# RaikoPipe/panda-gym

Measured on AMD Instinct MI355X. Metric: aggregate env-steps/s, PandaReach 4096 envs @1 GPU; 1/2/4/8-GPU scaling, higher is better.
Workload: dtype f32; 1 GPU; PandaReach-v3 (ee control, sparse reward), 4096 envs per GPU, the reference's scene: table / plane contacts of the robot (BASELINE configs[1]); envs_per_gpu=4096, global_envs=4096, parallelism=env-sharded x1

## Files before the change

panda-gym_amd/csrc/pgx_kernels.hip:

```cpp
#include <hip/hip_runtime.h>
#include <math.h>
#include <stdint.h>

#include "../../include/pgx.h"
#include "pgx_default_model.h"
#include "pgx_common.h"
#include "pgx_dev.h"
#include "pgx_model_consts.h"
#include "pgx_rows.h"

#ifdef PGX_PROF
#define PGX_PROF_N 24
__device__ unsigned long long pgx_prof_counters[PGX_PROF_N];
#define PGX_PROF_WAVES 16384
__device__ unsigned long long pgx_prof_wave[PGX_PROF_WAVES][10];
extern "C" int pgx_prof_wave_read(unsigned long long* out, int n) {
    return (int)hipMemcpyFromSymbol(out, HIP_SYMBOL(pgx_prof_wave), sizeof(unsigned long long) * 10 * (size_t)n);
}
extern "C" int pgx_prof_read(unsigned long long* out, int clear) {
    hipError_t e = hipMemcpyFromSymbol(out, HIP_SYMBOL(pgx_prof_counters), sizeof(unsigned long long) * PGX_PROF_N);
    if (e == hipSuccess && clear) {
        unsigned long long z[PGX_PROF_N] = {0};
        e = hipMemcpyToSymbol(HIP_SYMBOL(pgx_prof_counters), z, sizeof z);
    }
// ... 59 lines not shown
            printf("PGX_NAN tag %d sub %d block %d lane %d v %g %g %g %g %g %g %g | dt %g kp %g kd %g "     \
                   "maxv %g res %g erp %g fr %g it %d\n",                                                 \
                   (tag), (sub), (int)blockIdx.x, (int)threadIdx.x, (arr)[0], (n) > 1 ? (arr)[1] : 0.0f,   \
                   (n) > 2 ? (arr)[2] : 0.0f, (n) > 3 ? (arr)[3] : 0.0f, (n) > 4 ? (arr)[4] : 0.0f,        \
                   (n) > 5 ? (arr)[5] : 0.0f, (n) > 6 ? (arr)[6] : 0.0f, (mm).dt, (mm).kp, (mm).kd,         \
                   (mm).max_vel, (mm).residual_abs, (mm).contact_erp, (mm).friction, (mm).num_iterations); \
    } while (0)
#else
#define PGX_TRAP(tag, sub, arr, n, mm) ((void)0)
#endif

struct V3 {
    float x, y, z;
};
__device__ __forceinline__ V3 v3(float x, float y, float z) { return V3{x, y, z}; }
__device__ __forceinline__ V3 operator+(V3 a, V3 b) { return v3(a.x + b.x, a.y + b.y, a.z + b.z); }
__device__ __forceinline__ V3 operator-(V3 a, V3 b) { return v3(a.x - b.x, a.y - b.y, a.z - b.z); }
__device__ __forceinline__ V3 operator*(float s, V3 a) { return v3(s * a.x, s * a.y, s * a.z); }
__device__ __forceinline__ float dot(V3 a, V3 b) { return a.x * b.x + a.y * b.y + a.z * b.z; }
__device__ __forceinline__ V3 cross(V3 a, V3 b) {
    return v3(a.y * b.z - a.z * b.y, a.z * b.x - a.x * b.z, a.x * b.y - a.y * b.x);
}
__device__ __forceinline__ float fast_rcp(float x) { return __builtin_amdgcn_rcpf(x); }
__device__ __forceinline__ float fast_sqrt(float x) { return __builtin_amdgcn_sqrtf(x); }
__device__ __forceinline__ float norm(V3 a) { return fast_sqrt(dot(a, a)); }
__device__ __forceinline__ bool finite3(V3 a) {
    return __builtin_isfinite(a.x) && __builtin_isfinite(a.y) && __builtin_isfinite(a.z);
}

__device__ __forceinline__ void joint_sincos(float x, float* s_out, float* c_out) {
    const float k = rintf(x * 0.63661977236758134f);
    float r = fmaf(k, -1.5703125f, x);
    r = fmaf(k, -4.837512969970703125e-4f, r);
    r = fmaf(k, -7.54978995489188216e-8f, r);
    const float z = r * r;
    const float s = fmaf(r * z, fmaf(z, fmaf(z, -1.9515295891e-4f, 8.3321608736e-3f), -1.6666654611e-1f), r);
    const float c = fmaf(z * z, fmaf(z, fmaf(z, 2.443315711809948e-5f, -1.388731625493765e-3f), 4.166664568298827e-2f),
                         fmaf(-0.5f, z, 1.0f));
    const int q = (int)k & 3;
    const float ss = (q & 1) ? c : s, cc = (q & 1) ? s : c;
    *s_out = (q & 2) ? -ss : ss;
    *c_out = ((q + 1) & 2) ? -cc : cc;
}

template <int W>
__device__ __forceinline__ V3 lds3(const float (*a)[W], int ln) { return v3(a[0][ln], a[1][ln], a[2][ln]); }

typedef float f2 __attribute__((ext_vector_type(2)));
#ifndef PGX_PK
#define PGX_PK 4
#endif
#ifndef PGX_PK_AO
#define PGX_PK_AO 2
#endif
__device__ __forceinline__ void pk_fma_acc(float& a, float& b, f2 cab, float s) {
    const f2 r = __builtin_elementwise_fma(cab, (f2){s, s}, (f2){a, b});
    a = r.x;
    b = r.y;
}
constexpr int GW = 16;
constexpr int EPW = 64 / GW;

template <int V>
struct IC {
    static constexpr int value = V;
};
template <int B, int E, class F>
__device__ __forceinline__ void sfor(F&& f) {
    if constexpr (B < E) {
        f(IC<B>{});
        sfor<B + 1, E>(f);
    }
}
template <int CTRL>
__device__ __forceinline__ float dpp(float x) {
    return __builtin_bit_cast(float, __builtin_amdgcn_update_dpp(0, __builtin_bit_cast(int, x), CTRL, 0xF, 0xF, true));
}
template <int SRC>
__device__ __forceinline__ float bcast16(float x) {
    return dpp<0x150 + SRC>(x);
}
__device__ __forceinline__ float sum16(float x) {
    x += dpp<0xB1>(x);
    x += dpp<0x4E>(x);
    x += dpp<0x141>(x);
    x += dpp<0x140>(x);
    return x;
}
template <int K>
__device__ __forceinline__ float lane_sel(float a, float other) {
    constexpr uint64_t mask = 0x0001000100010001ull << K;
    float r;
    asm("v_cndmask_b32 %0, %1, %2, %3" : "=v"(r) : "v"(other), "v"(a), "s"(mask));
    return r;
}
__device__ __forceinline__ float pick_obj(V3 lin, V3 ang) {
    float v = 0.0f;
    v = lane_sel<7>(lin.x, v); v = lane_sel<8>(lin.y, v); v = lane_sel<9>(lin.z, v);
    v = lane_sel<10>(ang.x, v); v = lane_sel<11>(ang.y, v); v = lane_sel<12>(ang.z, v);
    return v;
}
__device__ __forceinline__ float pick_arm(const float* a, float other) {
    float v = other;
    sfor<0, NJ>([&](auto kc) __attribute__((always_inline)) { v = lane_sel<decltype(kc)::value>(a[decltype(kc)::value], v); });
    return v;
}
// ... 491 lines not shown
#ifndef PGX_CGR_OBJ
#define PGX_CGR_OBJ 6
#endif
#ifndef PGX_CGR_ARM
#define PGX_CGR_ARM 4
#endif
static_assert(PGX_CGR_ARM >= 2 && PGX_CGR_OBJ >= 2, "the sweeps' point counts are 0, 2, 4 (<= the register budget)");
template <int W, int OBJ, int FULL>
constexpr int robot_regs() {
    return (W != 64 && FULL) ? (OBJ ? PGX_CGR_OBJ : PGX_CGR_ARM) : CG;
}

constexpr int CACHE_N = 2 * PGX_CONTACT_SLOTS;
constexpr int CACHE1 = 2 * CG;
constexpr float kTableIdLimit = 32.0f;
static_assert(PGX_NCAP <= 16, "PgxDevModel.cap_mu holds 16 capsules");

template <int AO, int FULL = 0>
__device__ __forceinline__ float point_mu(MRef m, float id) {
    const float cf = id < kTableIdLimit ? id * 0.5f
                   : (id - kTableIdLimit) * (AO ? ((FULL && AO_PERS) ? (1.0f / 24.0f) : (1.0f / 6.0f)) : 0.0625f);
    const int cap = (int)(cf + 1e-3f);
    float mu = m.friction;
    sfor<0, PGX_NCAP>([&](auto kc) __attribute__((always_inline)) {
        constexpr int K = decltype(kc)::value;
        mu = cap == K ? m.cap_mu[K] : mu;
    });
    return mu;
}

template <int W, int OBJ = 1, int FULL = 0>
struct ContactLdsT {
    static constexpr int RB = robot_budget<W, OBJ, FULL>();
    static constexpr int P0 = OBJ ? CG : 0;
    static constexpr int CGR = robot_regs<W, OBJ, FULL>();
    static constexpr int NQR = 3 * (P0 + CGR), NQX = 3 * (P0 + RB);
    static constexpr int XR = (W == 64 || RB <= CGR) ? 1 : NQX - NQR;
    static constexpr int MP = (W == 64 || !FULL) ? 1 : (OBJ ? PGX_MANIFOLD_POOL : PGX_MANIFOLD_POOL_AO);
    static constexpr int G0 = (W == 64 || OBJ) ? CG : 1;
    float4 g0q[G0][4][W];
    float g0d[G0][W], g0id[G0][W];
    float g0n[G0][3][W];
    float g1p[RB][3][W];
    float g1n[RB][3][W];
    float g1rb[RB][3][W];
    float g1d[RB][W], g1id[RB][W];
    int g1j[RB][W];
    int g1w[RB][W];
    int mcnt[W];
    float mkid[MP][W], mla[MP][3][W], mlb[MP][3][W], mn[MP][3][W], md[MP][W], mimp[MP][W];
    float4 g1q[W == 64 ? CG : 1][3][6][W == 64 ? W : 1];
    int cnt[2][W];
    float cache[CACHE_N][W];
    float capA[PGX_NCAP][3][W], capB[PGX_NCAP][3][W];
    float aoC[PGX_AO_OBSTACLES][3][W];
    float aoD[PGX_AO_LINKS][W], aoU[PGX_AO_LINKS][3][W];
    float4 wJ[W == 64 ? 1 : W][W == 64 ? 1 : NQR][4], wR[W == 64 ? 1 : W][W == 64 ? 1 : NQR][2];
    float2 xd[(W == 64 || XR == 1) ? 1 : W][XR][16];
    float xrhs[XR][W], xlam[XR][W], xlam0[XR][W], xfk[XR][W], xjinv[XR][W];
    float pjn[W == 64 ? 1 : P0 + CGR][W], pl0[W == 64 ? 1 : P0 + CGR][W];
    float lrhs[(W == 64 || !OBJ) ? 1 : PGX_N_ROWS - PGX_NJ][W], llam[(W == 64 || !OBJ) ? 1 : PGX_N_ROWS - PGX_NJ][W];
    float ltq[W == 64 ? 1 : PGX_NJ][W], lqs[W == 64 ? 1 : 2][W == 64 ? 1 : PGX_NJ][W];
    float lkc[W == 64 ? 1 : 16][W == 64 ? 1 : 16];
    float psv[W == 64 ? 1 : 27][W == 64 ? 1 : W];
    float spec0[W == 64 ? NJ + 6 : 1][W == 64 ? W : 1];
};
using ContactLds = ContactLdsT<64>;
template <int OBJ, int FULL>
using ContactLdsGT = ContactLdsT<EPW, OBJ, FULL>;

template <int N, class LT>
__device__ __forceinline__ float warm_lookup(const LT& L, int ln, int first, float id, float factor) {
    float warm = 0.0f;
#pragma unroll
    for (int s = 0; s < N; s++) {
        const float sid = L.cache[first + 2 * s][ln], imp = L.cache[first + 2 * s + 1][ln];
        warm = sid == id ? factor * imp : warm;
    }
    return warm;
}

struct ObjState {
    V3 p, v, w;
    float qx, qy, qz, qw;
};

__device__ __forceinline__ void plane_space(V3 n, V3& p, V3& q) {
    if (fabsf(n.z) > 0.70710678f) {
        float a = n.y * n.y + n.z * n.z, k = __builtin_amdgcn_rsqf(a);
        p = v3(0.0f, -n.z * k, n.y * k);
        q = v3(a * k, -n.x * p.z, n.x * p.y);
    } else {
        float a = n.x * n.x + n.y * n.y, k = __builtin_amdgcn_rsqf(a);
        p = v3(-n.y * k, n.x * k, 0.0f);
        q = v3(-n.z * p.y, n.z * p.x, a * k);
    }
}

__device__ __forceinline__ bool on_table(const PgxDevEnv& e, float x, float y) {
    return fabsf(x - e.table_cx) <= e.table_hx && fabsf(y - e.table_cy) <= e.table_hy;
}
__device__ __forceinline__ float ground_z(const PgxDevEnv& e, float x, float y) {
    return on_table(e, x, y) ? e.table_top : e.plane_z;
}
__device__ __forceinline__ float vertex_vs_table(const PgxDevEnv& e, V3 P, V3& n) {
    const float bot = e.table_top - 2.0f * e.table_hz;
    const float qx = P.x - e.table_cx, qy = P.y - e.table_cy;
// ... 537 lines not shown
        const V3 A = v3(L.capA[c][0][ln], L.capA[c][1][ln], L.capA[c][2][ln]);
        const V3 B = v3(L.capB[c][0][ln], L.capB[c][1][ln], L.capB[c][2][ln]);
        const float r = kCapR[c];
        const int flags = kCapFlags[c], jc = kCapJ[c], ns = kCapNs[c];
        if (flags & PGX_CAP_VS_TABLE) {
            for (int end = 0; end < (ns == 1 ? 1 : 2); end++) {
                const V3 P = end ? B : A;
                const bool ont = on_table(e, P.x, P.y);
                const float zt = ont ? e.table_top : e.plane_z;
                const float d = P.z - r - zt;
                if (d < (ont ? cap_tau<TAU_TABLE>(m, c) : cap_tau<TAU_PLANE>(m, c)))
                    g1_insert(L, ln, d, (float)(2 * c + end), jc, v3(P.x, P.y, P.z - r), v3(0.0f, 0.0f, 1.0f),
                              v3(0.0f, 0.0f, 0.0f));
            }
        }
        if (OBJ && (flags & PGX_CAP_VS_OBJECT)) object_candidates(e, cap_tau<TAU_OBJ>(m, c), L, ln, ob, Rc, c, true);
        if (AO && flags != 0) {
            const float tau = cap_tau<TAU_OBST>(m, c);
            if (ao_capsule_near(L, ln, c, tau)) ao_obstacle_candidates(L, ln, c, tau);
        }
    }
}

template <int C = 0, class LT>
__device__ __forceinline__ void link_capsules(int j, LT& L, int ln, const M3& R, V3 oj) {
    if constexpr (C < PGX_NCAP) {
        if (kCapJ[C] == j) {
            const V3 A = oj + mulc(R, kCapA[C]), B = oj + mulc(R, kCapB[C]);
            L.capA[C][0][ln] = A.x; L.capA[C][1][ln] = A.y; L.capA[C][2][ln] = A.z;
            L.capB[C][0][ln] = B.x; L.capB[C][1][ln] = B.y; L.capB[C][2][ln] = B.z;
        }
        link_capsules<C + 1, LT>(j, L, ln, R, oj);
    }
}

struct CapLane {
    float r;
    int flags, ns, j, slot;
};
__device__ __forceinline__ CapLane cap_lane() {
    float r = kCapR[0], fl = (float)kCapFlags[0], ns = (float)kCapNs[0], j = (float)kCapJ[0];
    float sl = (float)ao_slot(0);
    sfor<1, PGX_NCAP>([&](auto kc) __attribute__((always_inline)) {
        constexpr int K = decltype(kc)::value;
        r = lane_sel<K>(kCapR[K], r);
        fl = lane_sel<K>((float)kCapFlags[K], fl);
        ns = lane_sel<K>((float)kCapNs[K], ns);
        j = lane_sel<K>((float)kCapJ[K], j);
        sl = lane_sel<K>((float)ao_slot(K), sl);
    });
    return CapLane{r, (int)fl, (int)ns, (int)j, (int)sl};
}

template <class LT>
__device__ __forceinline__ void robot_table_contacts_g(MRef m, const PgxDevEnv& e, LT& L, int es, int c) {
    const int cc = c < PGX_NCAP ? c : 0;
    const CapLane cl = cap_lane();
    const bool on = c < PGX_NCAP && (cl.flags & PGX_CAP_VS_TABLE);
    const V3 A = lds3(L.capA[cc], es), B = lds3(L.capB[cc], es);
    const float r = cl.r;
    const bool two = cl.ns != 1;
    const float tt = cap_tau<TAU_TABLE>(m, cc), tp = cap_tau<TAU_PLANE>(m, cc);
    const bool t0 = on_table(e, A.x, A.y), t1 = on_table(e, B.x, B.y);
    const float d0 = A.z - r - (t0 ? e.table_top : e.plane_z);
    const float d1 = B.z - r - (t1 ? e.table_top : e.plane_z);
    const bool c0 = on && d0 < (t0 ? tt : tp), c1 = on && two && d1 < (t1 ? tt : tp);
    unsigned m0 = row_ballot(c0), m1 = row_ballot(c1);
    const int total = __builtin_popcount(m0) + __builtin_popcount(m1);
    bool k0 = c0, k1 = c1;
    if (__any(total > LT::RB)) {
        const float e0 = c0 ? d0 : 3.0e38f, e1 = c1 ? d1 : 3.0e38f;
        int r0 = 0, r1 = 0;
        sfor<0, PGX_NCAP>([&](auto kc) __attribute__((always_inline)) {
            constexpr int K = decltype(kc)::value;
            const float y0 = bcast16<K>(e0), y1 = bcast16<K>(e1);
            r0 += (y0 < e0 || (y0 == e0 && K < c)) + (y1 < e0 || (y1 == e0 && K < c));
            r1 += (y0 < e1 || (y0 == e1 && K <= c)) + (y1 < e1 || (y1 == e1 && K < c));
        });
        k0 = c0 && r0 < LT::RB;
        k1 = c1 && r1 < LT::RB;
        m0 = row_ballot(k0);
        m1 = row_ballot(k1);
    }
    const unsigned below = (1u << (c & 15)) - 1u;
    const int base = __builtin_popcount(m0 & below) + __builtin_popcount(m1 & below);
    const int jc = cl.j;
    if (k0) {
        const int sl = base;
        L.g1d[sl][es] = d0; L.g1id[sl][es] = (float)(2 * c); L.g1j[sl][es] = jc; L.g1w[sl][es] = -1;
        L.g1p[sl][0][es] = A.x; L.g1p[sl][1][es] = A.y; L.g1p[sl][2][es] = A.z - r;
        L.g1n[sl][0][es] = 0.0f; L.g1n[sl][1][es] = 0.0f; L.g1n[sl][2][es] = 1.0f;
        L.g1rb[sl][0][es] = 0.0f; L.g1rb[sl][1][es] = 0.0f; L.g1rb[sl][2][es] = 0.0f;
    }
    if (k1) {
        const int sl = base + (k0 ? 1 : 0);
        L.g1d[sl][es] = d1; L.g1id[sl][es] = (float)(2 * c + 1); L.g1j[sl][es] = jc; L.g1w[sl][es] = -1;
        L.g1p[sl][0][es] = B.x; L.g1p[sl][1][es] = B.y; L.g1p[sl][2][es] = B.z - r;
        L.g1n[sl][0][es] = 0.0f; L.g1n[sl][1][es] = 0.0f; L.g1n[sl][2][es] = 1.0f;
        L.g1rb[sl][0][es] = 0.0f; L.g1rb[sl][1][es] = 0.0f; L.g1rb[sl][2][es] = 0.0f;
    }
    L.cnt[1][es] = __builtin_popcount(m0) + __builtin_popcount(m1);
}

struct Dyn {
    V3 z[NJ], o[NJ];
    float Mi[NJ][NJ];
    float mcol[NJ];
    float mdiag[NJ];
    float vu[NJ];
    V3 vcu, wcu;
    bool coll;
};

template <int OBJ, int CONT, class LT, bool PAR = false, int AO = 0>
__device__ __forceinline__ void substep_dyn(MRef m, const PgxDevEnv& e, const float* q, const float* qd,
                                            const ObjState& ob, LT* Lp, int ln, Dyn& D, int lane = 0) {
    M3 Rc;
    if (OBJ) Rc = quat_mat(ob);
    if (CONT) { Lp->cnt[0][ln] = 0; Lp->cnt[1][ln] = 0; }
    if (OBJ) {
        const float h = e.obj_half;
#pragma unroll
        for (int k = 0; k < 16; k++) {
            const int vtx = k & 7;
            const V3 r = mul(Rc, v3((vtx & 1) ? h : -h, (vtx & 2) ? h : -h, (vtx & 4) ? h : -h));
            const V3 P = ob.p + r;
            V3 n = v3(0.0f, 0.0f, 1.0f);
            const float d = k < 8 ? vertex_vs_table(e, P, n) : P.z - e.plane_z;
            if (d < (k < 8 ? m.tau_obj_table : m.tau_obj_plane)) g0_insert(*Lp, ln, d, (float)k, r, n);
        }
    }
    V3 (&z)[NJ] = D.z;
    V3 (&o)[NJ] = D.o;
    V3 c[NJ];
    S3 Iw[NJ];
    M3 R6;
    {
        M3 PR = {{1, 0, 0, 0, 1, 0, 0, 0, 1}};
        V3 PO = v3(m.base[0], m.base[1], m.base[2]);
        float sjs[NJ], cjs[NJ];
        joint_sincos_all<PAR>(q, sjs, cjs);
#pragma unroll
        for (int j = 0; j < NJ; j++) {
            M3 R = mulm(PR, kJr[j]);
            V3 oj = PO + mulc(PR, kJp[j]);
            const float s = sjs[j], cs = cjs[j];
#pragma unroll
            for (int r = 0; r < 3; r++) {
                float a = R.m[r * 3], b = R.m[r * 3 + 1];
                R.m[r * 3] = cs * a + s * b;
                R.m[r * 3 + 1] = -s * a + cs * b;
            }
            z[j] = col(R, 2);
            o[j] = oj;
// ... 93 lines not shown
            for (int i = 0; i < j; i++) Mt[j][i] = dot(z[i], n0 + cross(o[j] - o[i], f));
        }
    }
    chol7(Mt);
    float (&vu)[NJ] = D.vu;
    {
        float qdd[NJ];
        chol7_solve(Mt, nb, qdd);
#pragma unroll
        for (int j = 0; j < NJ; j++) vu[j] = fminf(fmaxf(qd[j] + m.dt * qdd[j], -m.max_vel), m.max_vel);
    }

    PGX_PROF_MARK(15);
    float (&Mi)[NJ][NJ] = D.Mi;
    {
        float X[NJ][NJ];
#pragma unroll
        for (int i = 0; i < NJ; i++) {
            float inv = Mt[i][i];
#pragma unroll
            for (int jj = 0; jj <= i; jj++) {
                float s = (jj == i) ? 1.0f : 0.0f;
#pragma unroll
                for (int kk = jj; kk < i; kk++) s -= Mt[i][kk] * X[kk][jj];
                X[i][jj] = s * inv;
            }
        }
#pragma unroll
        for (int i = 0; i < NJ; i++)
#pragma unroll
            for (int jj = 0; jj <= i; jj++) {
                float s = 0.0f;
#pragma unroll
                for (int l = i; l < NJ; l++) s += X[l][i] * X[l][jj];
                Mi[i][jj] = s;
            }
    }

    V3& vcu = D.vcu;
    V3& wcu = D.wcu;
    vcu = v3(0, 0, 0);
    wcu = v3(0, 0, 0);
    if (OBJ) {
        const float vn = norm(ob.v), wn = norm(ob.w);
        vcu = ob.v + m.dt * (g - (m.lin_damp + m.lin_damp * vn) * ob.v - cross(ob.w, ob.v));
        wcu = ob.w - (m.dt * (m.ang_damp + m.ang_damp * wn)) * ob.w;
    }
}

struct LaneK {
    float mass, com[3];
    float I[6], Iown[6];
};
__device__ __forceinline__ void lane_consts(LaneK& k) {
    k.mass = 0.0f;
#pragma unroll
    for (int t = 0; t < 3; t++) k.com[t] = 0.0f;
#pragma unroll
    for (int t = 0; t < 6; t++) { k.I[t] = 0.0f; k.Iown[t] = 0.0f; }
    sfor<0, NJ>([&](auto jc) __attribute__((always_inline)) {
        constexpr int j = decltype(jc)::value;
        k.mass = lane_sel<j>(kMass[j], k.mass);
#pragma unroll
        for (int t = 0; t < 3; t++) k.com[t] = lane_sel<j>(kCom[j][t], k.com[t]);
#pragma unroll
        for (int t = 0; t < 6; t++) {
            const float a = j < NJ - 1 ? (t < 3 ? kInertia[j < NJ - 1 ? j : 0][t < 3 ? t : 0] : 0.0f) : kI6c[t];
            const float b = j < NJ - 1 ? a : kI6own[t];
            if (a != 0.0f) k.I[t] = lane_sel<j>(a, k.I[t]);
            if (b != 0.0f) k.Iown[t] = lane_sel<j>(b, k.Iown[t]);
        }
    });
}
__device__ __forceinline__ float row_pre(float x) {
    x += dpp<0x111>(x);
    x += dpp<0x112>(x);
    x += dpp<0x114>(x);
    return x;
}
__device__ __forceinline__ float row_suf(float x) {
    x += dpp<0x101>(x);
    x += dpp<0x102>(x);
    x += dpp<0x104>(x);
    return x;
}
__device__ __forceinline__ V3 row_pre(V3 a) { return v3(row_pre(a.x), row_pre(a.y), row_pre(a.z)); }
__device__ __forceinline__ V3 row_suf(V3 a) { return v3(row_suf(a.x), row_suf(a.y), row_suf(a.z)); }
__device__ __forceinline__ float link_only(float x) {
    float r;
    asm("v_cndmask_b32 %0, 0, %1, %2" : "=v"(r) : "v"(x), "s"(0x007F007F007F007Full));
    return r;
}
__device__ __forceinline__ V3 link_only(V3 a) { return v3(link_only(a.x), link_only(a.y), link_only(a.z)); }
__device__ __forceinline__ S3 rot_sym_r(const M3& R, const float* s) {
    const float Sm[9] = {s[0], s[3], s[4], s[3], s[1], s[5], s[4], s[5], s[2]};
    float T[9];
#pragma unroll
    for (int i = 0; i < 3; i++)
#pragma unroll
        for (int j = 0; j < 3; j++)
            T[i * 3 + j] = R.m[i * 3] * Sm[j] + R.m[i * 3 + 1] * Sm[3 + j] + R.m[i * 3 + 2] * Sm[6 + j];
    auto e = [&](int i, int j) { return T[i * 3] * R.m[j * 3] + T[i * 3 + 1] * R.m[j * 3 + 1] + T[i * 3 + 2] * R.m[j * 3 + 2]; };
    S3 o;
    o.xx = e(0, 0); o.yy = e(1, 1); o.zz = e(2, 2); o.xy = e(0, 1); o.xz = e(0, 2); o.yz = e(1, 2);
    return o;
}
__device__ __forceinline__ V3 mul_sym(const float* s, V3 v) {
    return v3(s[0] * v.x + s[3] * v.y + s[4] * v.z, s[3] * v.x + s[1] * v.y + s[5] * v.z,
              s[4] * v.x + s[5] * v.y + s[2] * v.z);
}

template <int OBJ, int CONT, int AO = 0, int FULL = 0>
__device__ __forceinline__ void substep_dyn_g(MRef m, const PgxDevEnv& e, const float* q, const float* qd,
                                              const ObjState& ob, ContactLdsGT<OBJ, FULL>* Lp, int es, Dyn& D, int c,
                                              const LaneK& K, bool check = false) {
    M3 Rc;
    D.coll = false;
    if (OBJ) Rc = quat_mat(ob);
    if (CONT) { Lp->cnt[0][es] = 0; Lp->cnt[1][es] = 0; }
    if (OBJ) {
        const float h = e.obj_half;
        const int vtx = c & 7;
        const V3 r = mul(Rc, v3((vtx & 1) ? h : -h, (vtx & 2) ? h : -h, (vtx & 4) ? h : -h));
        const V3 P = ob.p + r;
        V3 nrm = v3(0.0f, 0.0f, 1.0f);
        const float d = c < 8 ? vertex_vs_table(e, P, nrm) : P.z - e.plane_z;
        const bool cand = d < (c < 8 ? m.tau_obj_table : m.tau_obj_plane);
        const float dd = cand ? d : 3.0e38f;
        int rank = 0;
        sfor<0, 16>([&](auto uc) __attribute__((always_inline)) {
            constexpr int U = decltype(uc)::value;
            const float du = bcast16<U>(dd);
            rank += (du < dd || (du == dd && U < c)) ? 1 : 0;
        });
        const bool keep = cand && rank < CG;
        const unsigned mk = row_ballot(keep);
        const int sl = __builtin_popcount(mk & ((1u << (c & 15)) - 1u));
        if (keep) {
            Lp->g0d[sl][es] = d;
            Lp->g0id[sl][es] = (float)c;
            Lp->g0q[sl][0][es] = make_float4(r.x, r.y, r.z, 0.0f);
            Lp->g0n[sl][0][es] = nrm.x; Lp->g0n[sl][1][es] = nrm.y; Lp->g0n[sl][2][es] = nrm.z;
        }
        Lp->cnt[0][es] = __builtin_popcount(mk);
        PGX_PROF_MARK(19);
    }
    V3 (&z)[NJ] = D.z;
    V3 (&o)[NJ] = D.o;
    M3 Rl = {{0, 0, 0, 0, 0, 0, 0, 0, 0}};
    V3 ol = v3(0, 0, 0);
    {
        M3 PR = {{1, 0, 0, 0, 1, 0, 0, 0, 1}};
        V3 PO = v3(m.base[0], m.base[1], m.base[2]);
        float sjs[NJ], cjs[NJ];
        joint_sincos_all<true>(q, sjs, cjs);
        sfor<0, NJ>([&](auto jc) __attribute__((always_inline)) {
            constexpr int j = decltype(jc)::value;
            M3 R = mulm(PR, kJr[j]);
            V3 oj = PO + mulc(PR, kJp[j]);
            const float sn = sjs[j], cs = cjs[j];
#pragma unroll
            for (int r = 0; r < 3; r++) {
                float a = R.m[r * 3], b = R.m[r * 3 + 1];
                R.m[r * 3] = cs * a + sn * b;
                R.m[r * 3 + 1] = -sn * a + cs * b;
            }
            z[j] = col(R, 2);
            o[j] = oj;
            if constexpr (CONT) link_capsules(j, *Lp, es, R, oj);
#pragma unroll
            for (int t = 0; t < 9; t++) Rl.m[t] = lane_sel<j>(R.m[t], Rl.m[t]);
            ol = v3(lane_sel<j>(oj.x, ol.x), lane_sel<j>(oj.y, ol.y), lane_sel<j>(oj.z, ol.z));
            PR = R;
            PO = oj;
        });
    }
    if (CONT) {
        if constexpr (!OBJ) {
            robot_table_contacts_g(m, e, *Lp, es, c);
            if constexpr (AO) {
                const int cc = c < PGX_NCAP ? c : 0;
                const float tau = cap_tau<TAU_OBST>(m, cc);
                const CapLane cl = cap_lane();
                const bool cap_on = c < PGX_NCAP && cl.flags != 0;
                const int slot = c < PGX_NCAP ? cl.slot : -1;
                const bool chk = check && slot >= 0;
                const V3 A = lds3(Lp->capA[cc], es), B = lds3(Lp->capB[cc], es);
                const float r = cl.r;
                const V3 hcube = v3(kAoSize, kAoSize, kAoSize);
                const int row0 = (int)(threadIdx.x & ~(unsigned)(GW - 1));
                bool sorted = false, hit = false;
                if (chk && slot >= 1) {
                    V3 tc = ao_table_c(e), th = ao_table_h(e);
                    asm volatile("" : "+v"(tc.x), "+v"(tc.y), "+v"(tc.z), "+v"(th.x), "+v"(th.y), "+v"(th.z));
                    const V3 thi = v3(th.x - kAoMargin, th.y - kAoMargin, th.z - kAoMargin);
                    const float lb = fminf(box_sd(A, tc, thi), box_sd(B, tc, thi)) - 0.5f * norm(B - A) - kAoMargin - r;
                    if (lb <= 0.0f) hit = capsule_box_hit(A, B, r, tc, th);
                }
                unsigned cmask = 0;
                int o1 = -1;
                V3 pa1 = v3(0.0f, 0.0f, 0.0f), pb1 = pa1, n1v = pa1;
                float d1 = 0.0f;
                V3 Cs[AO_N];
#pragma unroll
                for (int o = 0; o < AO_N; o++) Cs[o] = lds3(Lp->aoC[o], es);
#ifdef PGX_AB_NO_OBST
                if (true) {} else
#endif
#pragma unroll
                for (int o = 0; o < AO_N; o++) {
                    const V3 C = Cs[o];
                    V3 P = seg_closest(A, B, C);
                    const V3 v = C - P;
                    const float len = norm(v);
                    float d = 3.0e38f;
                    V3 n = len > 0.0f ? fast_rcp(len) * v : v3(0.0f, 0.0f, 1.0f);
                    if (cap_on || chk) {
                        if (o < 3) d = len - r - kAoSize;
                        else if (len - r - kAoCubeBound < (cap_on ? tau : 0.0f))
#ifdef PGX_AB_NO_BOXPAIR
                            d = len - r - kAoCubeBound;
#else
                            d = capsule_box_pair<true>(A, B, r, C, hcube, &P, &n);
#endif
                    }
                    hit = hit || (chk && d <= 0.0f);
                    const bool cand = cap_on && d < tau;
                    if constexpr (FULL && AO_PERS) {
                        cmask |= cand ? (1u << o) : 0u;
                        if (cand && o1 < 0) {
                            o1 = o;
                            pa1 = P + r * n;
// ... 86 lines not shown
            const uint64_t bn = __ballot(near);
            unsigned wm = (unsigned)((bn | (bn >> 16) | (bn >> 32) | (bn >> 48)) & 0xFFFFu);
            if constexpr (FULL) {
                const unsigned rm = row_ballot(near);
                wm = __builtin_amdgcn_readfirstlane(wm);
                while (wm) {
                    const int cn = __builtin_ctz(wm);
                    wm &= wm - 1u;
                    object_new_point_g(e, cap_tau<TAU_OBJ>(m, cn), *Lp, es, ob, Rc, cn, c, ((rm >> cn) & 1u) != 0, Rl, ol);
                }
                if (__any(Lp->mcnt[es] > 0)) man_refresh_insert_g<1, 0>(m, *Lp, es, c, Rl, ol, Rc, ob.p);
                PGX_PROF_MARK(21);
            } else if (wm) {
                const unsigned rm = row_ballot(near);
                sort_g1_by_depth(*Lp, es);
                wm = __builtin_amdgcn_readfirstlane(wm);
                while (wm) {
                    const int cn = __builtin_ctz(wm);
                    wm &= wm - 1u;
                    object_candidates_g(e, cap_tau<TAU_OBJ>(m, cn), *Lp, es, ob, Rc, cn, c, ((rm >> cn) & 1u) != 0);
                }
                PGX_PROF_MARK(21);
                sort_groups(*Lp, es);
            }
        }
    }
    PGX_PROF_MARK(1);
    const V3 g = v3(m.gravity[0], m.gravity[1], m.gravity[2]);
    const V3 base = v3(m.base[0], m.base[1], m.base[2]);
    const V3 zl = col(Rl, 2);
    const V3 ob_l = ol - base;
    const V3 cw = ol + mul(Rl, v3(K.com[0], K.com[1], K.com[2]));
    const V3 cb = cw - base;

    const float qdl = pick_arm(qd, 0.0f);
    const V3 t1 = qdl * zl;
    const V3 w = row_pre(t1);
    const V3 alt = cross(w - t1, t1);
    const V3 al = row_pre(alt);
    const V3 S = row_pre(cross(t1, ob_l));
    const V3 u = cross(w, ob_l) - S;
    const V3 dS = row_pre(cross(alt, ob_l) + cross(t1, u));
    const V3 v = cross(w, cb) - S;
    const V3 a = cross(al, cb) + cross(w, v) - dS;
    const S3 Iw = rot_sym_r(Rl, K.I);
    const V3 Iww = mul(Iw, w);
    const float wn = norm(w);
    const V3 Iow = mul(Rl, mul_sym(K.Iown, mul_t(Rl, w)));
    V3 F = K.mass * (a - g);
    V3 T = mul(Iw, al) + cross(w, Iww) + (m.ang_damp + m.ang_damp * wn) * Iow;
    {
        const V3 Fd = (K.mass * (m.lin_damp + m.lin_damp * norm(v))) * v;
        V3 Fg = v3(0, 0, 0), Tg = v3(0, 0, 0);
#pragma unroll
        for (int b = 0; b < PGX_NDAMP; b++) {
            const V3 rb = mulc(Rl, kDpos[b]);
            const V3 vb = u + cross(w, rb);
            const V3 fd = (kDmass[b] * (m.lin_damp + m.lin_damp * norm(vb))) * vb;
            Fg = Fg + fd;
            Tg = Tg + cross(ol + rb - cw, fd);
        }
        F = F + v3(lane_sel<NJ - 1>(Fg.x, Fd.x), lane_sel<NJ - 1>(Fg.y, Fd.y), lane_sel<NJ - 1>(Fg.z, Fd.z));
        T = T + v3(lane_sel<NJ - 1>(Tg.x, 0.0f), lane_sel<NJ - 1>(Tg.y, 0.0f), lane_sel<NJ - 1>(Tg.z, 0.0f));
    }
    const V3 Fs = row_suf(link_only(F));
    const V3 Ms = row_suf(link_only(T + cross(cb, F)));
    const float nbl = -dot(zl, Ms - cross(ob_l, Fs));
    PGX_PROF_MARK(14);

    float Mt[NJ][NJ], yb[NJ];
    {
        const float ml = link_only(K.mass);
        const S3 st = steiner(ml, cb);
        const float Mc = row_suf(ml);
        const V3 H = row_suf(ml * cb);
        const float Ixx = row_suf(link_only(Iw.xx + st.xx)), Iyy = row_suf(link_only(Iw.yy + st.yy));
        const float Izz = row_suf(link_only(Iw.zz + st.zz)), Ixy = row_suf(link_only(Iw.xy + st.xy));
        const float Ixz = row_suf(link_only(Iw.xz + st.xz)), Iyz = row_suf(link_only(Iw.yz + st.yz));
        const S3 Is = {Ixx, Iyy, Izz, Ixy, Ixz, Iyz};
        const V3 f = cross(zl, H - Mc * ob_l);
        const float Ho = dot(H, ob_l), oz = dot(ob_l, zl), Hz = dot(H, zl), oo = dot(ob_l, ob_l);
        const V3 n = mul(Is, zl) + (Mc * oo - 2.0f * Ho) * zl + oz * H + Hz * ob_l - (Mc * oz) * ob_l;
        float colv[NJ];
#pragma unroll
        for (int i = 0; i < NJ; i++) colv[i] = dot(z[i], n + cross(ol - o[i], f));
        chol7_rows(colv, nbl, Mt, yb);
    }
    float (&vu)[NJ] = D.vu;
    {
        float qdd[NJ];
        chol7_back(Mt, yb, qdd);
#pragma unroll
        for (int j = 0; j < NJ; j++) vu[j] = fminf(fmaxf(qd[j] + m.dt * qdd[j], -m.max_vel), m.max_vel);
    }

    PGX_PROF_MARK(15);
    {
        float y[NJ], x[NJ];
        sfor<0, NJ>([&](auto ic) __attribute__((always_inline)) {
            constexpr int i = decltype(ic)::value;
            float sacc = lane_sel<i>(1.0f, 0.0f);
#pragma unroll
            for (int k = 0; k < i; k++) sacc -= Mt[i][k] * y[k];
            y[i] = sacc * Mt[i][i];
        });
#pragma unroll
        for (int i = NJ - 1; i >= 0; i--) {
            float sacc = y[i];
#pragma unroll
            for (int k = i + 1; k < NJ; k++) sacc -= Mt[k][i] * x[k];
            x[i] = sacc * Mt[i][i];
        }
#pragma unroll
// ... 2185 lines not shown
        L->mcnt[ln] = mc;
        if (c < mc) {
            const float* b = s.man + (size_t)(1 + PGX_MANIFOLD_POINT * c) * N + ii;
            L->mkid[c][ln] = b[0];
#pragma unroll
            for (int t = 0; t < 3; t++) {
                L->mla[c][t][ln] = b[(size_t)(1 + t) * N];
                L->mlb[c][t][ln] = b[(size_t)(4 + t) * N];
                L->mn[c][t][ln] = b[(size_t)(7 + t) * N];
            }
            L->md[c][ln] = b[(size_t)10 * N];
            L->mimp[c][ln] = b[(size_t)11 * N];
        }
    }
    if constexpr (AO) ao_load(s, N, ii, *L, ln);

    const int A = e.action_dim;
    if (CONTROL == 0) {
        float a[3];
#pragma unroll
        for (int c = 0; c < 3; c++) a[c] = fminf(fmaxf(action[(size_t)ii * A + c], -1.0f), 1.0f);
        float qcl[NJ];
#pragma unroll
        for (int j = 0; j < NJ; j++) qcl[j] = s.qc[j * N + ii];
        Chain k;
        fk_chain<WIDE != 0>(m, qcl, k);
        V3 pos = k.o[NJ - 1] + mulc(k.R[NJ - 1], kEeCom);
        V3 tgt = pos + v3(a[0] * m.ee_step, a[1] * m.ee_step, a[2] * m.ee_step);
        tgt.z = fmaxf(0.0f, tgt.z);
        const float torn[4] = {1.0f, 0.0f, 0.0f, 0.0f};
        ik<WIDE != 0>(mp, q, tgt, torn, tq);
        if constexpr (!WIDE) PGX_TRAP(0, 0, tq, NJ, m);
    } else {
#pragma unroll
        for (int j = 0; j < NJ; j++) {
            float a = fminf(fmaxf(action[(size_t)ii * A + j], -1.0f), 1.0f);
            tq[j] = q[j] + a * m.joint_step;
        }
    }

    bool bad_in = false;
    if constexpr (GUARD) {
        bool fin = true;
#pragma unroll
        for (int j = 0; j < NJ; j++)
            fin = fin && __builtin_isfinite(q[j]) && __builtin_isfinite(qd[j]) && __builtin_isfinite(tq[j]);
        if constexpr (OBJ)
            fin = fin && finite3(ob.p) && finite3(ob.v) && finite3(ob.w) && __builtin_isfinite(ob.qx) &&
                  __builtin_isfinite(ob.qy) && __builtin_isfinite(ob.qz) && __builtin_isfinite(ob.qw);
        bad_in = !fin;
    }
    PGX_PROF_MARK(0);
    LaneK lk;
    if constexpr (WIDE) lane_consts(lk);
    const int n_substeps = e.n_substeps;
    bool collided = false;
    float qprev[NJ];
#pragma unroll
    for (int j = 0; j < NJ; j++) qprev[j] = q[j];
    constexpr bool PARK = WIDE && CONT && (OBJ || AO || PART == 2);
    auto lds_st = [&](float* a, float v) __attribute__((always_inline)) { __hip_atomic_store(a, v, __ATOMIC_RELAXED, __HIP_MEMORY_SCOPE_WAVEFRONT); };
    auto lds_ld = [&](float* a) __attribute__((always_inline)) { return __hip_atomic_load(a, __ATOMIC_RELAXED, __HIP_MEMORY_SCOPE_WAVEFRONT); };
    float* lkf = &lk.mass;
    static_assert(sizeof(LaneK) == 16 * sizeof(float), "LaneK layout");
    if constexpr (PARK) {
#pragma unroll
        for (int j = 0; j < NJ; j++) lds_st(&L->ltq[j][ln], tq[j]);
#pragma unroll
        for (int f = 0; f < 16; f++) lds_st(&L->lkc[f][c], lkf[f]);
    }
    int qslot = 0;
    for (int st = 0; st < n_substeps; st++) {
        float qstart[NJ];
        if constexpr (PARK) {
#pragma unroll
            for (int j = 0; j < NJ; j++) {
                lds_st(&L->lqs[st & 1][j][ln], q[j]);
                tq[j] = lds_ld(&L->ltq[j][ln]);
            }
#pragma unroll
            for (int f = 0; f < 16; f++) lkf[f] = lds_ld(&L->lkc[f][c]);
        } else {
#pragma unroll
            for (int j = 0; j < NJ; j++) qstart[j] = q[j];
        }
        if constexpr (WIDE) {
            int cl = c, esl = ln;
            if constexpr (AO) asm volatile("" : "+v"(cl), "+v"(esl));
            if (substep_g<OBJ, CONT, PART, AO, FULL>(mp, e, q, qd, tq, ob, L, esl, cl, lk, AO && st > 0)) {
                collided = true;
                break;
            }
        } else {
            substep<OBJ, CONT, AO>(mp, e, q, qd, tq, ob, L, ln);
        }
        if constexpr (PARK) qslot = st & 1;
        else {
#pragma unroll
            for (int j = 0; j < NJ; j++) qprev[j] = qstart[j];
        }
        if constexpr (AO && !WIDE) {
            ao_caps(*fresh(mp), q, *L, ln);
            if (ao_collided(e, *L, ln)) { collided = true; break; }
        }
    }
    if constexpr (AO && WIDE) {
        if (!collided) {
// ... 653 lines not shown
```

Before: 12.24 million env-steps/s.

## Compute capsule endpoints and damping bodies on idle row lanes via permutes

```diff
diff --git a/panda-gym_amd/csrc/pgx_kernels.hip b/panda-gym_amd/csrc/pgx_kernels.hip
--- a/panda-gym_amd/csrc/pgx_kernels.hip
+++ b/panda-gym_amd/csrc/pgx_kernels.hip
@@ -135,6 +135,12 @@
 #endif
 #ifndef PGX_PK_AO
 #define PGX_PK_AO 2
+#endif
+#ifndef PGX_OWN_CAPS
+#define PGX_OWN_CAPS 1
+#endif
+#ifndef PGX_OWN_DAMP
+#define PGX_OWN_DAMP 1
 #endif
 __device__ __forceinline__ void pk_fma_acc(float& a, float& b, f2 cab, float s) {
     const f2 r = __builtin_elementwise_fma(cab, (f2){s, s}, (f2){a, b});
@@ -732,7 +738,12 @@
     float4 g1q[W == 64 ? CG : 1][3][6][W == 64 ? W : 1];
     int cnt[2][W];
     float cache[CACHE_N][W];
-    float capA[PGX_NCAP][3][W], capB[PGX_NCAP][3][W];
+    union alignas(16) {
+        struct {
+            float capA[PGX_NCAP][3][W], capB[PGX_NCAP][3][W];
+        };
+        float capk[W == 64 ? 1 : GW][12];
+    };
     float aoC[PGX_AO_OBSTACLES][3][W];
     float aoD[PGX_AO_LINKS][W], aoU[PGX_AO_LINKS][3][W];
     float4 wJ[W == 64 ? 1 : W][W == 64 ? 1 : NQR][4], wR[W == 64 ? 1 : W][W == 64 ? 1 : NQR][2];
@@ -1376,15 +1387,100 @@
     return CapLane{r, (int)fl, (int)ns, (int)j, (int)sl};
 }
 
+__device__ __forceinline__ float pmul(float x, float k) { return x * k; }
+__device__ __forceinline__ V3 mull(const M3& A, const float* v) {
+    return v3(pmul(A.m[0], v[0]) + pmul(A.m[1], v[1]) + pmul(A.m[2], v[2]),
+              pmul(A.m[3], v[0]) + pmul(A.m[4], v[1]) + pmul(A.m[5], v[2]),
+              pmul(A.m[6], v[0]) + pmul(A.m[7], v[1]) + pmul(A.m[8], v[2]));
+}
+template <uint64_t MASK>
+__device__ __forceinline__ float mask_sel(float a, float other) {
+    float r;
+    asm("v_cndmask_b32 %0, %1, %2, %3" : "=v"(r) : "v"(other), "v"(a), "s"(MASK));
+    return r;
+}
+template <int N>
+constexpr uint64_t zero_lanes(const float (&T)[N][3], int t, int L0, int K0 = 0) {
+    uint64_t mk = 0;
+    for (int k = K0; k < N; k++)
+        if (T[k][t] == 0.0f) mk |= 0x0001000100010001ull << (L0 + k);
+    return mk;
+}
+template <uint64_t Z0, uint64_t Z1, uint64_t Z2>
+__device__ __forceinline__ void own_cols(M3& R) {
+#pragma unroll
+    for (int r = 0; r < 3; r++) {
+        if constexpr (Z0 != 0) R.m[3 * r] = mask_sel<Z0>(-1.0f, R.m[3 * r]);
+        if constexpr (Z1 != 0) R.m[3 * r + 1] = mask_sel<Z1>(-1.0f, R.m[3 * r + 1]);
+        if constexpr (Z2 != 0) R.m[3 * r + 2] = mask_sel<Z2>(-1.0f, R.m[3 * r + 2]);
+    }
+}
+struct CapEnds {
+    float a[3], b[3];
+};
+__device__ __forceinline__ CapEnds cap_ends_lane() {
+    CapEnds k = {{0.0f, 0.0f, 0.0f}, {0.0f, 0.0f, 0.0f}};
+    sfor<1, PGX_NCAP>([&](auto kc) __attribute__((always_inline)) {
+        constexpr int K = decltype(kc)::value;
+        static_assert(kCapJ[K] >= 0 && kCapJ[K] < NJ, "lane kCapJ[c] of the row holds capsule c's frame");
+#pragma unroll
+        for (int t = 0; t < 3; t++) {
+            if (kCapA[K][t] != 0.0f) k.a[t] = lane_sel<K>(kCapA[K][t], k.a[t]);
+            if (kCapB[K][t] != 0.0f) k.b[t] = lane_sel<K>(kCapB[K][t], k.b[t]);
+        }
+    });
+    return k;
+}
+struct CapRow {
+    CapEnds k;
+    CapLane cl;
+    float tt, tp;
+    int src4;
+};
+typedef float f4 __attribute__((ext_vector_type(4)));
 template <class LT>
-__device__ __forceinline__ void robot_table_contacts_g(MRef m, const PgxDevEnv& e, LT& L, int es, int c) {
+__device__ __forceinline__ void cap_row_fill(MRef m, LT& L, int c) {
+    static_assert(sizeof(L.capk) <= sizeof(L.capA) + sizeof(L.capB), "the rows fit where the end points were");
     const int cc = c < PGX_NCAP ? c : 0;
     const CapLane cl = cap_lane();
+    const CapEnds k = cap_ends_lane();
+    f4* row = reinterpret_cast<f4*>(L.capk[c]);
+    row[0] = (f4){k.a[0], k.a[1], k.a[2], cl.r};
+    row[1] = (f4){k.b[0], k.b[1], k.b[2], __int_as_float(cl.flags | (cl.ns << 8) | ((cl.j + 1) << 16))};
+    row[2] = (f4){cap_tau<TAU_TABLE>(m, cc), cap_tau<TAU_PLANE>(m, cc), __int_as_float((cl.j > 0 ? cl.j : 0) << 2), 0.0f};
+}
+template <class LT>
+__device__ __forceinline__ CapRow cap_row_load(LT& L, int c) {
+    const auto* row = (const volatile __attribute__((address_space(3))) f4*)(L.capk[c]);
+    const f4 a = row[0], b = row[1], t = row[2];
+    const int fl = __float_as_int(b.w);
+    return CapRow{{{a.x, a.y, a.z}, {b.x, b.y, b.z}}, CapLane{a.w, fl & 255, (fl >> 8) & 255, (fl >> 16) - 1, 0},
+                  t.x, t.y, __float_as_int(t.z)};
+}
+__device__ __forceinline__ void cap_ends_own(const M3& Rl, V3 ol, const CapRow& cr, V3& A, V3& B) {
+    static_assert(PGX_NCAP <= GW, "one capsule per lane of the row");
+    constexpr uint64_t ZA0 = zero_lanes(kCapA, 0, 0, 1), ZA1 = zero_lanes(kCapA, 1, 0, 1), ZA2 = zero_lanes(kCapA, 2, 0, 1);
+    static_assert(ZA0 == zero_lanes(kCapB, 0, 0, 1) && ZA1 == zero_lanes(kCapB, 1, 0, 1) && ZA2 == zero_lanes(kCapB, 2, 0, 1),
+                  "both ends of a capsule have the same zero components");
+    const int src = (int)((threadIdx.x & 63u & ~(unsigned)(GW - 1)) << 2) + cr.src4;
+    auto from = [&](float x) __attribute__((always_inline)) {
+        return __builtin_bit_cast(float, __builtin_amdgcn_ds_bpermute(src, __builtin_bit_cast(int, x)));
+    };
+    M3 R;
+#pragma unroll
+    for (int t = 0; t < 9; t++) R.m[t] = from(Rl.m[t]);
+    const V3 o = v3(from(ol.x), from(ol.y), from(ol.z));
+    own_cols<ZA0, ZA1, ZA2>(R);
+    A = o + mull(R, cr.k.a);
+    B = o + mull(R, cr.k.b);
+}
+
+template <class LT>
+__device__ __forceinline__ void robot_table_contacts_g(const PgxDevEnv& e, LT& L, int es, int c, V3 A, V3 B,
+                                                       const CapLane& cl, float tt, float tp) {
     const bool on = c < PGX_NCAP && (cl.flags & PGX_CAP_VS_TABLE);
-    const V3 A = lds3(L.capA[cc], es), B = lds3(L.capB[cc], es);
     const float r = cl.r;
     const bool two = cl.ns != 1;
-    const float tt = cap_tau<TAU_TABLE>(m, cc), tp = cap_tau<TAU_PLANE>(m, cc);
     const bool t0 = on_table(e, A.x, A.y), t1 = on_table(e, B.x, B.y);
     const float d0 = A.z - r - (t0 ? e.table_top : e.plane_z);
     const float d1 = B.z - r - (t1 ? e.table_top : e.plane_z);
@@ -1424,6 +1520,12 @@
         L.g1rb[sl][0][es] = 0.0f; L.g1rb[sl][1][es] = 0.0f; L.g1rb[sl][2][es] = 0.0f;
     }
     L.cnt[1][es] = __builtin_popcount(m0) + __builtin_popcount(m1);
+}
+template <class LT>
+__device__ __forceinline__ void robot_table_contacts_g(MRef m, const PgxDevEnv& e, LT& L, int es, int c) {
+    const int cc = c < PGX_NCAP ? c : 0;
+    robot_table_contacts_g(e, L, es, c, lds3(L.capA[cc], es), lds3(L.capB[cc], es), cap_lane(), cap_tau<TAU_TABLE>(m, cc),
+                           cap_tau<TAU_PLANE>(m, cc));
 }
 
 struct Dyn {
@@ -1623,6 +1725,7 @@
     float mass, com[3];
     float I[6], Iown[6];
 };
+template <bool DAMP = false>
 __device__ __forceinline__ void lane_consts(LaneK& k) {
     k.mass = 0.0f;
 #pragma unroll
@@ -1642,6 +1745,16 @@
             if (b != 0.0f) k.Iown[t] = lane_sel<j>(b, k.Iown[t]);
         }
     });
+    if constexpr (DAMP) {
+        static_assert(PGX_NDAMP <= GW - NJ, "one damping body per idle lane of the row");
+        sfor<0, PGX_NDAMP>([&](auto bc) __attribute__((always_inline)) {
+            constexpr int b = decltype(bc)::value;
+            k.mass = lane_sel<NJ + b>(kDmass[b], k.mass);
+#pragma unroll
+            for (int t = 0; t < 3; t++)
+                if (kDpos[b][t] != 0.0f) k.com[t] = lane_sel<NJ + b>(kDpos[b][t], k.com[t]);
+        });
+    }
 }
 __device__ __forceinline__ float row_pre(float x) {
     x += dpp<0x111>(x);
@@ -1685,6 +1798,7 @@
 __device__ __forceinline__ void substep_dyn_g(MRef m, const PgxDevEnv& e, const float* q, const float* qd,
                                               const ObjState& ob, ContactLdsGT<OBJ, FULL>* Lp, int es, Dyn& D, int c,
                                               const LaneK& K, bool check = false) {
+    constexpr bool OWN_CAPS = PGX_OWN_CAPS && CONT && !OBJ && !AO, OWN_DAMP = PGX_OWN_DAMP && !OBJ && !AO;
     M3 Rc;
     D.coll = false;
     if (OBJ) Rc = quat_mat(ob);
@@ -1738,7 +1852,7 @@
             }
             z[j] = col(R, 2);
             o[j] = oj;
-            if constexpr (CONT) link_capsules(j, *Lp, es, R, oj);
+            if constexpr (CONT && !OWN_CAPS) link_capsules(j, *Lp, es, R, oj);
 #pragma unroll
             for (int t = 0; t < 9; t++) Rl.m[t] = lane_sel<j>(R.m[t], Rl.m[t]);
             ol = v3(lane_sel<j>(oj.x, ol.x), lane_sel<j>(oj.y, ol.y), lane_sel<j>(oj.z, ol.z));
@@ -1748,7 +1862,14 @@
     }
     if (CONT) {
         if constexpr (!OBJ) {
-            robot_table_contacts_g(m, e, *Lp, es, c);
+            if constexpr (OWN_CAPS) {
+                const CapRow cr = cap_row_load(*Lp, c);
+                V3 A, B;
+                cap_ends_own(Rl, ol, cr, A, B);
+                robot_table_contacts_g(e, *Lp, es, c, A, B, cr.cl, cr.tt, cr.tp);
+            } else {
+                robot_table_contacts_g(m, e, *Lp, es, c);
+            }
             if constexpr (AO) {
                 const int cc = c < PGX_NCAP ? c : 0;
                 const float tau = cap_tau<TAU_OBST>(m, cc);
@@ -1941,13 +2062,38 @@
     {
         const V3 Fd = (K.mass * (m.lin_damp + m.lin_damp * norm(v))) * v;
         V3 Fg = v3(0, 0, 0), Tg = v3(0, 0, 0);
-#pragma unroll
-        for (int b = 0; b < PGX_NDAMP; b++) {
-            const V3 rb = mulc(Rl, kDpos[b]);
-            const V3 vb = u + cross(w, rb);
-            const V3 fd = (kDmass[b] * (m.lin_damp + m.lin_damp * norm(vb))) * vb;
-            Fg = Fg + fd;
-            Tg = Tg + cross(ol + rb - cw, fd);
+        if constexpr (OWN_DAMP) {
+            constexpr int S = NJ - 1;
+            constexpr uint64_t Z0 = zero_lanes(kDpos, 0, NJ), Z1 = zero_lanes(kDpos, 1, NJ);
+            static_assert(Z0 == Z1 && zero_lanes(kDpos, 2, NJ) == 0, "a damping body is on the z axis or off both others");
+            float rbv[3];
+#pragma unroll
+            for (int r = 0; r < 3; r++) {
+                const float xy = pmul(bcast16<S>(Rl.m[3 * r]), K.com[0]) + pmul(bcast16<S>(Rl.m[3 * r + 1]), K.com[1]);
+                rbv[r] = (Z0 != 0 ? mask_sel<Z0>(-0.0f, xy) : xy) + pmul(bcast16<S>(Rl.m[3 * r + 2]), K.com[2]);
+            }
+            const V3 rb = v3(rbv[0], rbv[1], rbv[2]);
+            const V3 o6 = v3(bcast16<S>(ol.x), bcast16<S>(ol.y), bcast16<S>(ol.z));
+            const V3 c6 = v3(bcast16<S>(cw.x), bcast16<S>(cw.y), bcast16<S>(cw.z));
+            const V3 u6 = v3(bcast16<S>(u.x), bcast16<S>(u.y), bcast16<S>(u.z));
+            const V3 w6 = v3(bcast16<S>(w.x), bcast16<S>(w.y), bcast16<S>(w.z));
+            const V3 vb = u6 + cross(w6, rb);
+            const V3 fd = (K.mass * (m.lin_damp + m.lin_damp * norm(vb))) * vb;
+            const V3 td = cross(o6 + rb - c6, fd);
+            sfor<0, PGX_NDAMP>([&](auto bc) __attribute__((always_inline)) {
+                constexpr int b = NJ + decltype(bc)::value;
+                Fg = Fg + v3(bcast16<b>(fd.x), bcast16<b>(fd.y), bcast16<b>(fd.z));
+                Tg = Tg + v3(bcast16<b>(td.x), bcast16<b>(td.y), bcast16<b>(td.z));
+            });
+        } else {
+#pragma unroll
+            for (int b = 0; b < PGX_NDAMP; b++) {
+                const V3 rb = mulc(Rl, kDpos[b]);
+                const V3 vb = u + cross(w, rb);
+                const V3 fd = (kDmass[b] * (m.lin_damp + m.lin_damp * norm(vb))) * vb;
+                Fg = Fg + fd;
+                Tg = Tg + cross(ol + rb - cw, fd);
+            }
         }
         F = F + v3(lane_sel<NJ - 1>(Fg.x, Fd.x), lane_sel<NJ - 1>(Fg.y, Fd.y), lane_sel<NJ - 1>(Fg.z, Fd.z));
         T = T + v3(lane_sel<NJ - 1>(Tg.x, 0.0f), lane_sel<NJ - 1>(Tg.y, 0.0f), lane_sel<NJ - 1>(Tg.z, 0.0f));
@@ -4239,7 +4385,8 @@
     }
     PGX_PROF_MARK(0);
     LaneK lk;
-    if constexpr (WIDE) lane_consts(lk);
+    if constexpr (WIDE) lane_consts<PGX_OWN_DAMP && !OBJ && !AO>(lk);
+    if constexpr (WIDE && CONT && !OBJ && !AO && PGX_OWN_CAPS) cap_row_fill(*fresh(mp), *L, c);
     const int n_substeps = e.n_substeps;
     bool collided = false;
     float qprev[NJ];
```

Measured after the change: 12.80 million env-steps/s, median of 6. 4.6% higher.
